# Edresson/VoiceSplit

Measured on AMD Instinct MI355X. Metric: utterances/sec (3 s clips, B=64/GPU) fwd+bwd, channels-last bf16 activations / tape, bf16 MFMA, fp32 accumulate / statistics / master weights, higher is better.
Workload: dtype bf16 (conv activations and tape stored as bf16; bf16 MFMA operands in the convs, the LSTM / head contractions and the BPTT, f16 operands in the forward recurrence; fp32 accumulate, BatchNorm statistics, gate arithmetic / cell state, loss head, master weights)

## Files before the change

include/voicesplit_hip.h:

```cpp
#ifndef VOICESPLIT_HIP_H
#define VOICESPLIT_HIP_H

#include <stddef.h>
#include <stdint.h>

#ifdef __cplusplus
extern "C" {
#endif
#if defined(__GNUC__)
#pragma GCC visibility push(default)
#endif

#define VS_ABI_VERSION 11

#define VS_ACT_RELU 0
#define VS_ACT_MISH 1
#define VS_ACT_NONE 2
#define VS_ACT_SIGMOID 3

#define VS_MATH_FP32 0
#define VS_MATH_F16X3 1
#define VS_MATH_BF16 2

#define VS_BN_EVAL 0
// ... 257 lines not shown
                     int conv_act, int bn_mode, void* tape, size_t tape_bytes, float* mask, void* stream);

int vs_backward(const vs_dims* dims, const vs_params* params, const float* x, const float* dvec,
                int conv_act, int bn_mode, void* tape, size_t tape_bytes,
                const float* mask, const float* dmask, const vs_grads* grads, void* stream);

int vs_conv64_pack_dgrad(const float* w, float* packed, int KT, int KF, void* stream);
size_t vs_conv64_wgrad_partial_floats(int KT, int KF);
int vs_conv64_wgrad(const float* dz, const float* in, float* partials, float* dw,
                    int B, int T, int F, int KT, int KF, int dil, void* stream);
int vs_conv64_wgrad_f16x3(const float* dz, const float* in, float* partials, float* dw, float* scratch8,
                          int B, int T, int F, int KT, int KF, int dil, void* stream);
int vs_set_wgrad_kernel(int mode);
int vs_set_conv_kernel(int mode);
int vs_set_lstm_kernel(int mode);

enum vs_option {
  VS_OPT_FWD_PROLOGUE = 0,
  VS_OPT_HEAD_LEAF_SIDE = 1,
  VS_OPT_FEAT_ROWS = 2,
  VS_OPT_HEAD_BWD_GEMM = 3,
  VS_OPT_ABLATION = 4,
  VS_OPT_DETERMINISTIC = 5,
  VS_OPT_COUNT = 6
};
int vs_set_option(int option, int value);
int vs_get_option(int option);

int vs_lstm_status(const vs_dims* dims, const void* tape, size_t tape_bytes, const void* workspace, size_t workspace_bytes, void* stream);

int vs_set_backward_overlap(int on);
int vs_bn_act_bwd(const float* da, const float* z, float* dz, int C, long long R, int L, int act, int bn_mode,
                  const float* scale, const float* shift, const float* mean, const float* invstd,
                  float* dgamma, float* dbeta, float* dbias, double* stats, float* coef, void* stream);
int vs_bn_act_bwd_first(const float* da, const float* z, const float* x, float* xpad, int B, int T, int F, int act, int bn_mode,
                        const float* scale, const float* shift, const float* mean, const float* invstd,
                        float* dgamma, float* dbeta, float* dbias, float* dw, double* stats, float* coef, double* acc, void* stream);
int vs_conv_last_dgrad(const float* dz, const float* w, float* din, int B, int T, int F, void* stream);
int vs_conv_last_wgrad_blocks(void);
int vs_conv_last_wgrad(const float* dz, const float* in, float* partials , float* dw,
                       int B, int T, int F, void* stream);
int vs_conv_first_wgrad(const float* dz, const float* x, double* acc, float* dw, int B, int T, int F, void* stream);
int vs_gemm(int layout_a, int layout_w, const float* A, int lda, const float* W, int ldw, float* C, int ldc,
            int M, int N, int K, const float* bias, const float* gate, int ldg, int a_relu, int w_relu, int act,
            int accumulate, int w_shift, int w_group, int splits, float* partials, void* stream);
int vs_gemm_f16x3(int layout_a, int layout_w, const float* A, int lda, const float* W, int ldw, float* C, int ldc,
                  int M, int N, int K, const float* bias, const float* gate, int ldg, int a_relu, int w_relu, int act,
// ... 123 lines not shown
```

voicesplit_amd/_lib.py:

```python
import ctypes
import os
from ctypes import POINTER, Structure, c_char_p, c_float, c_int, c_longlong, c_size_t, c_void_p

_HERE = os.path.dirname(os.path.abspath(__file__))
LIB_PATH = os.path.join(_HERE, "libvoicesplit_hip.so")

ACT_RELU, ACT_MISH, ACT_NONE, ACT_SIGMOID = 0, 1, 2, 3
BN_EVAL, BN_TRAIN = 0, 1
MATH_FP32, MATH_F16X3, MATH_BF16 = 0, 1, 2
PROF_SLOTS = 29
PROF_NAMES = ("cnn1", "cnn2", "cnn3", "cnn4", "cnn5", "cnn6", "cnn7", "cnn8", "lstm_gemm", "lstm_rec", "head",
              "fwd_bn", "bwd_head", "bwd_lstm_rec", "bwd_lstm_gemm", "bwd_bn",
              "wgrad_cnn2", "wgrad_cnn3", "wgrad_cnn4", "wgrad_cnn5", "wgrad_cnn6", "wgrad_cnn7",
              "dgrad_cnn2", "dgrad_cnn3", "dgrad_cnn4", "dgrad_cnn5", "dgrad_cnn6", "dgrad_cnn7", "bwd_edge")
ABI_VERSION = 11


class VsDims(Structure):
    _fields_ = [(n, c_int) for n in ("B", "T", "F", "E", "H", "FC1", "FC2", "math")]


class VsConvLayer(Structure):
    _fields_ = [(n, c_void_p) for n in ("weight", "bias", "bn_weight", "bn_bias",
                                        "bn_running_mean", "bn_running_var")]
# ... 215 lines not shown


def load(path: str = None) -> ctypes.CDLL:
    global _lib
    if _lib is not None and path is None:
        return _lib
    path = path or LIB_PATH
    if not os.path.isfile(path):
        raise VoiceSplitHipError(
            f"{path} not found: build it with `python -c 'import __graft_entry__ as g; g.build()'` "
            f"or `make -C voicesplit_amd/csrc`. There is no PyTorch/CPU fallback for this path.")
    lib = ctypes.CDLL(path)
    for name, (restype, argtypes) in SIGNATURES.items():
        fn = getattr(lib, name)
        fn.restype = restype
        fn.argtypes = argtypes
    if lib.vs_abi_version() != ABI_VERSION:
        raise VoiceSplitHipError(f"{path}: ABI version {lib.vs_abi_version()} != {ABI_VERSION}; rebuild")
    _apply_env_options(lib)
    _lib = lib
    return lib


OPTIONS = {"FWD_PROLOGUE": 0, "HEAD_LEAF_SIDE": 1, "FEAT_ROWS": 2, "HEAD_BWD_GEMM": 3, "ABLATION": 4, "DETERMINISTIC": 5}
_ENV_OPTIONS = {
    "VOICESPLIT_FWD_PROLOGUE": ("FWD_PROLOGUE", int),
    "VOICESPLIT_HEAD_LEAF_SIDE": ("HEAD_LEAF_SIDE", int),
    "VOICESPLIT_FEAT_ROWS": ("FEAT_ROWS", int),
    "VOICESPLIT_HEAD_BWD_GEMM": ("HEAD_BWD_GEMM", int),
    "VOICESPLIT_ABLATION": ("ABLATION", int),
    "VOICESPLIT_DETERMINISTIC": ("DETERMINISTIC", int),
}


def _apply_env_options(lib):
    for var, (name, conv) in _ENV_OPTIONS.items():
        v = os.environ.get(var)
        if v is None or v == "":
            continue
        try:
            value = conv(v)
        except ValueError as err:
            raise VoiceSplitHipError(f"{var}={v}: not a value of this switch ({err})") from None
        if lib.vs_set_option(OPTIONS[name], value) != 0:
            msg = lib.vs_last_error()
            raise VoiceSplitHipError(f"{var}={v}: {msg.decode() if msg else 'rejected by vs_set_option'}")


def set_option(name: str, value: int):
    lib = load()
    prev = lib.vs_get_option(OPTIONS[name])
    check(lib.vs_set_option(OPTIONS[name], int(value)), f"vs_set_option({name})")
    return prev

# ... 10 lines not shown
```

voicesplit_amd/csrc/capi.hip:

```cpp
#include <stdarg.h>
#include <stdlib.h>
#include <string.h>

#include "../../include/voicesplit_hip.h"
#include "vs_internal.h"

static thread_local char g_err[512] = "";

void vs_set_error(const char* fmt, ...) {
  va_list ap;
  va_start(ap, fmt);
  vsnprintf(g_err, sizeof(g_err), fmt, ap);
  va_end(ap);
}

int g_vs_options[VS_OPT_COUNT] = { 1,  1,  1,  1,  0,  0};
thread_local unsigned* g_vs_turn = nullptr;

namespace {
struct Prof {
  bool on = false;
  int max_calls = 0;
  int calls[VS_PROF_SLOTS] = {0};
  hipEvent_t* ev = nullptr;
} g_prof;

}

VsProfScope::VsProfScope(int slot, hipStream_t s_) : s(s_), idx(-1) {
  if (!g_prof.on || g_prof.calls[slot] >= g_prof.max_calls) return;
  idx = (g_prof.calls[slot]++ * VS_PROF_SLOTS + slot) * 2;
  (void)hipEventRecord(g_prof.ev[idx], s);
}
VsProfScope::~VsProfScope() { if (idx >= 0) (void)hipEventRecord(g_prof.ev[idx + 1], s); }

extern "C" {

int vs_abi_version(void) { return VS_ABI_VERSION; }

// ... 396 lines not shown
```

voicesplit_amd/csrc/gemm_bf16.hip:

```cpp
#include <stdlib.h>

#include <type_traits>

#include "vs_internal.h"

namespace {

typedef unsigned u4v __attribute__((ext_vector_type(4)));
typedef short s4v __attribute__((ext_vector_type(4)));
typedef short s8v __attribute__((ext_vector_type(8)));
typedef __attribute__((address_space(3))) unsigned char lds_byte;
typedef __attribute__((address_space(3))) const u4v lds_u4v;

__device__ u4v g_gemm_zero_page[4];

constexpr int TM = 256, TN = 256, BK = 64;
constexpr int A_BYTES = TM * BK * 2;
constexpr int B_BYTES = TN * BK * 2;
constexpr int STAGE_BYTES = A_BYTES + B_BYTES;
constexpr int NSTAGE = 2;
constexpr int WA = 8, WB = 8;

struct GemmBf16Args {
  const unsigned short* A; int lda;
  const unsigned short* B; int ldb;
  float* C; int ldc;
  float* C2; int split_m;
  int M, N, K;
  const float* rowbias; int ldrb, group;
  int accumulate;
  int tiles_m, tiles_n, band;
  const float* gate; int ldg;
  int vec_ok;
};

__device__ __forceinline__ void glds16(const void* gsrc, unsigned lds_dst) {
  unsigned keep;
  asm volatile("s_mov_b32 %0, m0\n\ts_mov_b32 m0, %2\n\ts_nop 0\n\tglobal_load_lds_dwordx4 %1, off\n\ts_mov_b32 m0, %0"
               : "=&s"(keep) : "v"(gsrc), "s"(lds_dst) : "memory");
}
__device__ __forceinline__ vs_bf16x8 frag_of(s4v lo, s4v hi) {
  const s8v v = {lo[0], lo[1], lo[2], lo[3], hi[0], hi[1], hi[2], hi[3]};
  return __builtin_bit_cast(vs_bf16x8, v);
}
__device__ __forceinline__ s4v ds_read_tr16(unsigned addr) {
  return __builtin_amdgcn_ds_read_tr16_b64_v4i16((__attribute__((address_space(3))) s4v*)(uintptr_t)addr);
}

template <bool KMAJOR, int R>
struct Operand {
  static_assert(R == 256, "the lane decomposition below is for 256-row operand tiles");
  static constexpr int CHUNKS = R / 8 / 4;
  struct LaneDma { unsigned off[2]; int line; int col[2]; };
  __device__ static __forceinline__ LaneDma lane_dma(int ld, int wave, int lane) {
    LaneDma L;
    if (!KMAJOR) {
// ... 187 lines not shown
        const float* rb = g.rowbias ? g.rowbias + (size_t)(m / g.group) * g.ldrb : nullptr;
#pragma unroll
        for (int b = 0; b < WB; ++b) {
          const int n = tn * TN + wn * 128 + b * 16 + i;
          if (n < g.N) {
            float v = acc[a][b][r];
            if (rb) v += rb[n];
            if (g.accumulate) v += crow[n];
            if (g.gate) v = g.gate[(size_t)m * g.ldg + n] > 0.f ? v : 0.f;
            crow[n] = v;
          }
        }
      }
  }
}

__device__ __forceinline__ f32x4 acc_read(const f32x4& t) {
  f32x4 v;
  asm volatile("v_accvgpr_read_b32 %0, %4\n\tv_accvgpr_read_b32 %1, %5\n\tv_accvgpr_read_b32 %2, %6\n\tv_accvgpr_read_b32 %3, %7"
               : "=v"(v[0]), "=v"(v[1]), "=v"(v[2]), "=v"(v[3]) : "a"(t[0]), "a"(t[1]), "a"(t[2]), "a"(t[3]));
  return v;
}

template <bool AK, bool BK_, int DR, int ABL = 0>
__global__ __launch_bounds__(256, 1)
void gemm_bf16_il_kernel(GemmBf16Args g) {
  __shared__ __attribute__((aligned(16))) unsigned char smem[NSTAGE * STAGE_BYTES];
  using OA = Operand<AK, TM>;
  using OB = Operand<BK_, TN>;
  const int lane = threadIdx.x & 63;
  const int wave = __builtin_amdgcn_readfirstlane(threadIdx.x >> 6);
  const int wm = wave >> 1, wn = wave & 1;
  const unsigned lds0 = (unsigned)(uintptr_t)(const lds_byte*)smem;
  const int nk = (g.K + BK - 1) / BK;

  const int per = (int)(gridDim.x >> 3);
  const int ntiles = g.tiles_m * g.tiles_n;
  const int tpx = (ntiles + 7) / 8;
  const int xcd = (int)(blockIdx.x & 7), slot = (int)(blockIdx.x >> 3);
  auto tile_id = [&](int j) { return xcd * tpx + slot + j * per; };
  auto tile_ok = [&](int j) { const int t = tile_id(j); return slot + j * per < tpx && t < ntiles; };

  int pj = 0, pk = 0, ptm = 0, ptn = 0;
  bool plive = tile_ok(0) && tile_of(g, tile_id(0), ptm, ptn);
  int pstage = 0;
  const unsigned fbA = AK ? (OA::frag_base(lane) ^ (unsigned)((wm * 8) << 5)) : (OA::frag_base(lane) + (unsigned)(wm * 128 * 128));
  const unsigned fbB = BK_ ? (OB::frag_base(lane) ^ (unsigned)((wn * 8) << 5)) : (OB::frag_base(lane) + (unsigned)(wn * 128 * 128));
  const typename OA::LaneDma la = OA::lane_dma(g.lda, wave, lane);
  const typename OB::LaneDma lb = OB::lane_dma(g.ldb, wave, lane);
  const unsigned pitchA = OA::chunk_pitch(g.lda), pitchB = OB::chunk_pitch(g.ldb);
  const unsigned kstepA = AK ? (unsigned)BK * (unsigned)g.lda * 2u : (unsigned)BK * 2u;
  const unsigned kstepB = BK_ ? (unsigned)BK * (unsigned)g.ldb * 2u : (unsigned)BK * 2u;
  const bool feed = g.accumulate >= 0;
  u4v dA = OA::tile_desc(g.A, g.lda, g.M, g.K, ptm * TM, 0, plive && feed), dB = OB::tile_desc(g.B, g.ldb, g.N, g.K, ptn * TN, 0, plive && feed);
  unsigned soffA = 0, soffB = 0;
  unsigned dstA = lds0 + (unsigned)(wave * 1024);
  auto dma_load = [&](unsigned voff, const u4v& desc, unsigned soff) {
    asm volatile("buffer_load_dwordx4 %0, %1, %2 offen lds" :: "v"(voff), "s"(desc), "s"(soff) : "memory");
  };
  auto adv = [&](u4v& d, unsigned step) {
    const unsigned long long b = (((unsigned long long)d[1] << 32) | d[0]) + step;
    d[0] = (unsigned)b;
    d[1] = (unsigned)(b >> 32);
    d[2] -= step;
  };
  auto pf_done = [&]() {
    pstage ^= 1;
    dstA = lds0 + (unsigned)(pstage * STAGE_BYTES) + (unsigned)(wave * 1024);
    if (++pk == nk) {
      pk = 0;
      ++pj;
      plive = tile_ok(pj) && tile_of(g, tile_id(pj), ptm, ptn);
      dA = OA::tile_desc(g.A, g.lda, g.M, g.K, ptm * TM, 0, plive && feed);
      dB = OB::tile_desc(g.B, g.ldb, g.N, g.K, ptn * TN, 0, plive && feed);
    }
  };
  if (plive) {
#pragma unroll
    for (int c = 0; c < 8; ++c) {
      asm volatile("s_mov_b32 m0, %0\n\ts_nop 0" :: "s"(dstA + (unsigned)(c * 4096)) : "memory");
      dma_load(AK ? la.off[c & 1] : la.off[0], dA, soffA);
      soffA += pitchA;
      asm volatile("s_mov_b32 m0, %0\n\ts_nop 0" :: "s"(dstA + (unsigned)(A_BYTES + c * 4096)) : "memory");
      dma_load(BK_ ? lb.off[c & 1] : lb.off[0], dB, soffB);
      soffB += pitchB;
    }
    soffA = soffB = 0;
    adv(dA, kstepA);
    adv(dB, kstepB);
    pf_done();
  }

  int cstage = 0;
  vs_bf16x8 bf[2][WB], afc, afn;
  asm volatile("s_waitcnt vmcnt(0)" ::: "memory");
  __builtin_amdgcn_s_barrier();
  for (int j = 0; tile_ok(j); ++j) {
    int tm, tn;
    if (!tile_of(g, tile_id(j), tm, tn)) break;
    f32x4 acc[WA][WB];
#pragma unroll
    for (int a = 0; a < WA; ++a)
#pragma unroll
      for (int b = 0; b < WB; ++b) acc[a][b] = f32x4{0.f, 0.f, 0.f, 0.f};
    {
      unsigned fa = lds0 + (unsigned)(cstage * STAGE_BYTES) + fbA, fb = lds0 + (unsigned)(cstage * STAGE_BYTES + A_BYTES) + fbB;
      asm volatile("" : "+v"(fa), "+v"(fb));
#pragma unroll
      for (int b = 0; b < WB; ++b) bf[0][b] = OB::frag(fb, b * 16, 0);
      afc = OA::frag(fa, 0, 0);
      afn = afc;
    }
    for (int ks = 0; ks < nk; ++ks) {
      const unsigned lv = (unsigned)__builtin_amdgcn_readfirstlane(plive ? 1 : 0);
      const unsigned stepA = (feed ? lv : 0u) * kstepA, stepB = (feed ? lv : 0u) * kstepB;
      unsigned fa = lds0 + (unsigned)(cstage * STAGE_BYTES) + fbA, fb = lds0 + (unsigned)(cstage * STAGE_BYTES + A_BYTES) + fbB;
      unsigned fan = lds0 + (unsigned)((cstage ^ 1) * STAGE_BYTES) + fbA, fbn = lds0 + (unsigned)((cstage ^ 1) * STAGE_BYTES + A_BYTES) + fbB;
      asm volatile("" : "+v"(fa), "+v"(fb), "+v"(fan), "+v"(fbn));
      const unsigned dstB = dstA + (unsigned)A_BYTES;
      __builtin_amdgcn_sched_barrier(0);
      auto row = [&](auto RC) {
        constexpr int R = decltype(RC)::value;
        constexpr int kh = R >> 3, a = R & 7;
        if (R == 15) {
          if (!(ABL & 2)) {
            asm volatile("s_waitcnt vmcnt(0) lgkmcnt(0)" ::: "memory");
            __builtin_amdgcn_s_barrier();
          }
          __builtin_amdgcn_sched_barrier(0);
        }
#pragma unroll
        for (int b = 0; b < WB; ++b) {
          asm volatile("v_mfma_f32_16x16x32_bf16 %0, %2, %1, %0" : "+a"(acc[a][b]) : "v"(afc), "v"(bf[kh][b]));
          if (ABL & 1) {
          } else if (R < 15) {
            if (b == 0) afn = (a + 1 < WA) ? OA::frag(fa, (a + 1) * 16, kh) : OA::frag(fa, 0, 1);
            if (kh == 0 && b == 1) bf[1][a] = OB::frag(fb, a * 16, 1);
          } else {
            bf[0][b] = OB::frag(fbn, b * 16, 0);
            if (b == WB - 1) afn = OA::frag(fan, 0, 0);
          }
          if (kh == 0 && DR == 8) {
            if (b == 2) asm volatile("s_add_i32 m0, %0, %1" :: "s"(dstA), "n"(a * 4096) : "scc", "memory");
            if (b == 3) dma_load(AK ? la.off[a & 1] : la.off[0], dA, soffA);
            if (b == 4) { soffA += pitchA; asm volatile("s_add_i32 m0, %0, %1" :: "s"(dstB), "n"(a * 4096) : "scc", "memory"); }
            if (b == 5) dma_load(BK_ ? lb.off[a & 1] : lb.off[0], dB, soffB);
            if (b == 6) soffB += pitchB;
          } else if (kh == 0 && DR == 4) {
            if (a < 4) {
              constexpr int c0 = (2 * a) & 7, c1 = (2 * a + 1) & 7;
              if (b == 0) asm volatile("s_add_i32 m0, %0, %1" :: "s"(dstA), "n"(c0 * 4096) : "scc", "memory");
              if (b == 1) { dma_load(AK ? la.off[c0 & 1] : la.off[0], dA, soffA); soffA += pitchA; }
              if (b == 2) asm volatile("s_add_i32 m0, %0, %1" :: "s"(dstB), "n"(c0 * 4096) : "scc", "memory");
              if (b == 3) { dma_load(BK_ ? lb.off[c0 & 1] : lb.off[0], dB, soffB); soffB += pitchB; }
              if (b == 4) asm volatile("s_add_i32 m0, %0, %1" :: "s"(dstA), "n"(c1 * 4096) : "scc", "memory");
              if (b == 5) { dma_load(AK ? la.off[c1 & 1] : la.off[0], dA, soffA); soffA += pitchA; }
              if (b == 6) asm volatile("s_add_i32 m0, %0, %1" :: "s"(dstB), "n"(c1 * 4096) : "scc", "memory");
              if (b == 7) { dma_load(BK_ ? lb.off[c1 & 1] : lb.off[0], dB, soffB); soffB += pitchB; }
            }
          } else {
            if (a == 0 && b == 2) adv(dA, stepA);
            if (a == 1 && b == 2) adv(dB, stepB);
          }
          __builtin_amdgcn_sched_barrier(0);
        }
        afc = afn;
      };
      row(std::integral_constant<int, 0>{});  row(std::integral_constant<int, 1>{});  row(std::integral_constant<int, 2>{});
      row(std::integral_constant<int, 3>{});  row(std::integral_constant<int, 4>{});  row(std::integral_constant<int, 5>{});
// ... 4 lines not shown
      soffA = soffB = 0;
      if (lv) pf_done();
      cstage ^= 1;
    }
    asm volatile("s_nop 15\n\ts_nop 15" ::: "memory");
    const int i = lane & 15, gq = lane >> 4;
    const bool whole = g.vec_ok && tm * TM + TM <= g.M && tn * TN + TN <= g.N;
    const int n0 = tn * TN + wn * 128 + 4 * gq;
    auto bias_ptr = [&](int a) -> const float* {
      int m = tm * TM + wm * 128 + a * 16 + i;
      m = m < g.M ? m : g.M - 1;
      return g.rowbias + (size_t)(m / g.group) * g.ldrb + n0;
    };
    f32x4 bias_nx[WB];
    if (whole && g.rowbias) {
      const float* rb0 = bias_ptr(0);
#pragma unroll
      for (int b = 0; b < WB; ++b) bias_nx[b] = *reinterpret_cast<const f32x4*>(rb0 + 16 * b);
    }
#pragma unroll
    for (int a = 0; a < WA; ++a) {
      const int m = tm * TM + wm * 128 + a * 16 + i;
      const int mc = m < g.M ? m : g.M - 1;
      float* crow = ((g.C2 && mc >= g.split_m) ? g.C2 + (size_t)(mc - g.split_m) * g.ldc : g.C + (size_t)mc * g.ldc) + n0;
      const float* rb = g.rowbias ? g.rowbias + (size_t)(mc / g.group) * g.ldrb + n0 : nullptr;
      if (whole) {
        f32x4 v[WB];
#pragma unroll
        for (int b = 0; b < WB; ++b) v[b] = acc_read(acc[a][b]);
        if (rb) {
#pragma unroll
          for (int b = 0; b < WB; ++b) v[b] += bias_nx[b];
          if (a + 1 < WA) {
            const float* rbn = bias_ptr(a + 1);
#pragma unroll
            for (int b = 0; b < WB; ++b) bias_nx[b] = *reinterpret_cast<const f32x4*>(rbn + 16 * b);
          }
        }
        if (g.accumulate > 0) {
#pragma unroll
          for (int b = 0; b < WB; ++b) v[b] += *reinterpret_cast<const f32x4*>(crow + 16 * b);
        }
        if (g.gate) {
          const float* gr = g.gate + (size_t)mc * g.ldg + n0;
#pragma unroll
          for (int b = 0; b < WB; ++b) {
            const f32x4 gt = *reinterpret_cast<const f32x4*>(gr + 16 * b);
// ... 51 lines not shown
      const f4 a0 = __builtin_nontemporal_load(p0), b0 = __builtin_nontemporal_load(p0 + 1);
      const f4 a1 = __builtin_nontemporal_load(p1), b1 = __builtin_nontemporal_load(p1 + 1);
      conv(i, a0, b0);
      conv(i + stride, a1, b1);
    }
    if (i < total) {
      const f4* p0 = addr(i);
      conv(i, __builtin_nontemporal_load(p0), __builtin_nontemporal_load(p0 + 1));
    }
    return;
  }
  for (long long i = (long long)blockIdx.x * 256 + threadIdx.x; i < total; i += (long long)gridDim.x * 256) {
    const long long r = i / groups;
    const int k0 = (int)(i - r * groups) * 8;
    const float* p = src + r * ld + k0;
    float x[8];
#pragma unroll
    for (int e = 0; e < 8; ++e) x[e] = (k0 + e < K) ? p[e] : 0.f;
    const u4v o = {vs_pack_bf16(x[0], x[1]), vs_pack_bf16(x[2], x[3]), vs_pack_bf16(x[4], x[5]), vs_pack_bf16(x[6], x[7])};
    *reinterpret_cast<u4v*>(dst + r * Kp + k0) = o;
  }
}

int gemm_cus() {
  int dev = 0, v = 0;
  if (hipGetDevice(&dev) != hipSuccess) return 256;
  if (hipDeviceGetAttribute(&v, hipDeviceAttributeMultiprocessorCount, dev) != hipSuccess || v <= 0) v = 256;
  return v;
}

}

int vs_cvt_rows_bf16_impl(const float* src, long long rows, int K, int ld, void* dst, int Kp, hipStream_t stream) {
  VS_REQUIRE(src && dst && rows > 0 && K > 0 && ld >= K && Kp >= K && Kp % 8 == 0, "cvt_rows_bf16: bad argument");
  const long long total = rows * (Kp >> 3);
  const long long nb = (total + 255) / 256;
  const long long ccap = 1LL << 24;
  const bool vec = K % 8 == 0 && ld % 4 == 0 && (reinterpret_cast<uintptr_t>(src) & 15) == 0 && (reinterpret_cast<uintptr_t>(dst) & 15) == 0;
  if (vec) hipLaunchKernelGGL(cvt_rows_bf16_kernel<true>, dim3((unsigned)(nb < ccap ? nb : ccap)), dim3(256), 0, stream, src, rows, K, ld,
                              reinterpret_cast<unsigned short*>(dst), Kp);
  else
  hipLaunchKernelGGL(cvt_rows_bf16_kernel<false>, dim3((unsigned)(nb < ccap ? nb : ccap)), dim3(256), 0, stream, src, rows, K, ld,
                     reinterpret_cast<unsigned short*>(dst), Kp);
  VS_LAUNCH_CHECK();
  return 0;
}

int vs_gemm_bf16_impl(int a_kmajor, int b_kmajor, const void* A, int lda, const void* B, int ldb, float* C, int ldc, float* C2, int split_m,
                      int M, int N, int K, const float* rowbias, int ldrb, int group, int accumulate, hipStream_t stream,
                      const float* gate, int ldg) {
  VS_REQUIRE(A && B && C && M > 0 && N > 0 && K > 0, "gemm_bf16: bad argument");
  VS_REQUIRE(lda % 8 == 0 && ldb % 8 == 0 && (reinterpret_cast<uintptr_t>(A) & 15) == 0 && (reinterpret_cast<uintptr_t>(B) & 15) == 0,
             "gemm_bf16: operands must be 16-byte aligned with ld a multiple of 8");
  VS_REQUIRE(!rowbias || (group > 0 && ldrb >= N), "gemm_bf16: rowbias needs group > 0 and ldrb >= N");
  VS_REQUIRE(!gate || (ldg >= N && !C2), "gemm_bf16: gate needs ldg >= N and a single output");
  VS_REQUIRE(a_kmajor || lda >= (K + BK - 1) / BK * BK, "gemm_bf16: row-form A must be padded to a multiple of %d in k", BK);
  VS_REQUIRE(b_kmajor || ldb >= (K + BK - 1) / BK * BK, "gemm_bf16: row-form B must be padded to a multiple of %d in k", BK);
  GemmBf16Args g{reinterpret_cast<const unsigned short*>(A), lda, reinterpret_cast<const unsigned short*>(B), ldb, C, ldc, C2, split_m,
                 M, N, K, rowbias, ldrb, group > 0 ? group : 1, accumulate, (M + TM - 1) / TM, (N + TN - 1) / TN, 8, gate, ldg, 0};
  g.vec_ok = N % 4 == 0 && ldc % 4 == 0 && (reinterpret_cast<uintptr_t>(C) & 15) == 0 && (!C2 || (reinterpret_cast<uintptr_t>(C2) & 15) == 0) &&
             (!rowbias || (ldrb % 4 == 0 && (reinterpret_cast<uintptr_t>(rowbias) & 15) == 0)) &&
             (!gate || (ldg % 4 == 0 && (reinterpret_cast<uintptr_t>(gate) & 15) == 0));
  static int cus = gemm_cus();
  const long long ntiles = (long long)g.tiles_m * g.tiles_n;
  long long nwg = cus / 8 * 8;
  if (nwg > (ntiles + 7) / 8 * 8) nwg = (ntiles + 7) / 8 * 8;
  if (nwg < 8) nwg = 8;
  const dim3 grid((unsigned)nwg), block(256);
  const int form = (!a_kmajor && !b_kmajor) ? 0 : (!a_kmajor && b_kmajor) ? 1 : (a_kmajor && b_kmajor) ? 2 : 3;
  VS_REQUIRE(form != 3, "gemm_bf16: the col x row form is not used by the path");
  if (g.vec_ok) {
#ifdef VS_ABLATION
    const int abl = vs_opt(VS_OPT_ABLATION);
    if (abl == 9) g.accumulate = -1;
    if (abl >= 1 && abl <= 3 && form == 0) {
      if (abl == 1) hipLaunchKernelGGL((gemm_bf16_il_kernel<false, false, 8, 1>), grid, block, 0, stream, g);
      else if (abl == 2) hipLaunchKernelGGL((gemm_bf16_il_kernel<false, false, 8, 2>), grid, block, 0, stream, g);
      else hipLaunchKernelGGL((gemm_bf16_il_kernel<false, false, 8, 3>), grid, block, 0, stream, g);
      VS_LAUNCH_CHECK();
      return 0;
    }
#endif
    if (form == 0) hipLaunchKernelGGL((gemm_bf16_il_kernel<false, false, 8>), grid, block, 0, stream, g);
    else if (form == 1) hipLaunchKernelGGL((gemm_bf16_il_kernel<false, true, 8>), grid, block, 0, stream, g);
    else hipLaunchKernelGGL((gemm_bf16_il_kernel<true, true, 8>), grid, block, 0, stream, g);
    VS_LAUNCH_CHECK();
    return 0;
  }
  if (form == 0) hipLaunchKernelGGL((gemm_bf16_kernel<false, false, 1>), grid, block, 0, stream, g);
  else if (form == 1) hipLaunchKernelGGL((gemm_bf16_kernel<false, true, 2>), grid, block, 0, stream, g);
  else hipLaunchKernelGGL((gemm_bf16_kernel<true, true, 2>), grid, block, 0, stream, g);
  VS_LAUNCH_CHECK();
  return 0;
// ... 2 lines not shown
```

voicesplit_amd/csrc/train.hip:

```cpp
#include <mutex>
#include <stdlib.h>
#include <string.h>

#include "../../include/voicesplit_hip.h"
#include "vs_internal.h"

namespace {

constexpr int kSplitK = 16;

inline size_t max3(size_t a, size_t b, size_t c) { return a > b ? (a > c ? a : c) : (b > c ? b : c); }

int tape_layout(const vs_dims* d, vs_tape_layout* L) {
  if (int rc = vs_check_dims_impl(d)) return rc;
  memset(L, 0, sizeof(*L));
  const size_t B = d->B, T = d->T, F = d->F, H = d->H, M = B * T;
  size_t off = 0;
  auto take = [&](size_t bytes) { size_t o = off; off = align_up(off + bytes); return o; };
  const size_t act = B * 64 * T * F * (d->math == VS_MATH_BF16 ? 2 : 4);
  for (int l = 0; l < 7; ++l) { L->z[l] = take(d->math == VS_MATH_BF16 && l == 0 ? 256 : act); L->a[l] = take(act); }
  L->z8 = take(M * 8 * F * 4);
  L->feat = take(M * 8 * F * 4);
  L->bn_scale = take(8 * 64 * 4);
  L->bn_shift = take(8 * 64 * 4);
  L->bn_mean = take(8 * 64 * 4);
  L->bn_invstd = take(8 * 64 * 4);
  L->gates = take(M * 8 * H * 4);
  L->cstate = take(M * 2 * H * 4);
  L->lstm_out = take(M * 2 * H * 4);
  L->fc1_out = take(M * (size_t)d->FC1 * 4);
  L->dlogits = take(M * (size_t)d->FC2 * 4);
  L->dfc1 = take(M * (size_t)d->FC1 * 4);
  L->dlstm_out = take(M * 2 * H * 4);
  L->dsum = take(B * 8 * H * 4);
  L->dfeat = take(M * 8 * F * 4);
  L->grad0 = take(act);
  L->grad1 = take(act);
  L->dvbias = take(B * 8 * H * 4);
  for (int i = 0; i < 6; ++i) L->conv_packed[i] = take(vs_conv64_packed_floats(kMid[i].kt, kMid[i].kf) * 4);
  L->pack_tmp = take(vs_conv64_packed_floats(5, 5) * 4);
  L->lstm_packed = take(vs_lstm_packed_floats(d->H) * 4);
  L->lstm_packed_t = take(vs_lstm_packed_t_floats(d->H) * 4);
  L->lstm_state = take(vs_lstm_state_floats(d->B, d->H) * 4);
  L->lstm_bwd_state = take(vs_lstm_bwd_state_floats(d->B, d->H) * 4);
  L->consts = take(128 * 4);
  L->bn_stats = take((size_t)VS_BN_STAT_SLOTS * 64 * 2 * 8);
  L->bn_coef = take(3 * 64 * 4);
  L->first_acc = take((64 + VS_FIRST_BWD_SCRATCH_DOUBLES) * 8);
  L->colsum_tmp = take(2 * B * max3(8 * H, d->FC1, d->FC2) * 4);
  size_t part = vs_conv64_wgrad_partial_floats(5, 5);
  part = max3(part, vs_conv64_wgrad_partial_floats(7, 1), (size_t)vs_conv_last_wgrad_blocks() * 512);
  part = max3(part, (size_t)kSplitK * d->FC2 * d->FC1, (size_t)kSplitK * d->FC1 * 2 * H);
  part = max3(part, (size_t)kSplitK * 4 * H * H, (size_t)0);
  L->partials = take(part * 4);
  L->conv_scales = take(16 * VS_SCALE_SLOT_FLOATS * 4);
  L->gemm_scales = take(32 * 4);
  L->lstm_bf16 = take(d->math == VS_MATH_BF16 ? vs_lstm_bf16_layout((long long)M, 8 * (int)F, (int)H).total : 256);
  L->det_turn = take(VS_TURN_WORDS * 4 + (size_t)VS_BN_STAT_SLOTS * 576 * 8);
  for (int i = 0; i < 6; ++i) L->conv_packed_t[i] = take(vs_conv64_packed_floats(kMid[i].kt, kMid[i].kf) * 4);
  L->total_bytes = off;
  return 0;
}

int check_tape(const vs_dims* d, void* tape, size_t bytes, vs_tape_layout* L) {
  if (int rc = tape_layout(d, L)) return rc;
  VS_REQUIRE(tape != nullptr, "tape is NULL");
  VS_REQUIRE((reinterpret_cast<uintptr_t>(tape) & 255) == 0, "tape must be 256-byte aligned");
  VS_REQUIRE(bytes >= L->total_bytes, "tape too small: %zu < %zu bytes", bytes, L->total_bytes);
  return 0;
}

int check_params(const vs_params* p) {
  VS_REQUIRE(p != nullptr, "params is NULL");
  for (int l = 0; l < 8; ++l) {
    const vs_conv_layer& c = p->conv[l];
    VS_REQUIRE(c.weight && c.bias && c.bn_weight && c.bn_bias && c.bn_running_mean && c.bn_running_var,
               "conv layer %d has a NULL parameter", l + 1);
  }
  for (int dir = 0; dir < 2; ++dir)
    VS_REQUIRE(p->w_ih[dir] && p->w_hh[dir] && p->b_ih[dir] && p->b_hh[dir], "NULL LSTM parameter (dir %d)", dir);
// ... 363 lines not shown
                                      st.B, st.T, st.H, st.stream, st.d->math);
}

int lstm_leaves(const Step& st, const SideJoin& sj, const float* dvec, const vs_grads* g) {
  hipStream_t ls = sj.to();
  const vs_params* p = st.p;
  const vs_tape_layout& L = st.L;
  const int B = st.B, T = st.T, H = st.H, M = st.M, K8 = st.K8, KE = st.KE, E = st.d->E;
  const bool f16x3 = st.d->math == VS_MATH_F16X3;
  float* dxg = st.at<float>(L.gates);
  float* dsum = st.at<float>(L.dsum);
  float* feat = st.at<float>(L.feat);
  float* lstm_out = st.at<float>(L.lstm_out);
  float* tmp = st.at<float>(L.colsum_tmp);
  float* gsc = st.at<float>(L.gemm_scales);
  char* bfb = st.at<char>(L.lstm_bf16);
  auto dwih_bf16 = [&]() -> int {
    return vs_gemm_bf16_impl(1, 1, bfb + st.lb.dxg, 8 * H, bfb + st.lb.feat, st.lb.Kp, g->w_ih[0], KE, g->w_ih[1], 4 * H, 8 * H, K8, M, nullptr, 0, 1, 0, ls);
  };
  const bool wih_last = sj.side != nullptr;
  VsProfScope ps(VS_PROF_BWD_LSTM_GEMM, ls);
  if (int rc = vs_colsum_impl(dxg, 8 * H, B, T, 8 * H, dsum, 8 * H, ls)) return rc;
  if (int rc = vs_colsum_impl(dsum, 8 * H, 1, B, 8 * H, tmp, 8 * H, ls)) return rc;
  for (int dir = 0; dir < 2; ++dir) {
    VS_CHECK_HIP(hipMemcpyAsync(g->b_ih[dir], tmp + (size_t)dir * 4 * H, sizeof(float) * 4 * H, hipMemcpyDeviceToDevice, ls));
    VS_CHECK_HIP(hipMemcpyAsync(g->b_hh[dir], tmp + (size_t)dir * 4 * H, sizeof(float) * 4 * H, hipMemcpyDeviceToDevice, ls));
    const float* dxg_d = dxg + (size_t)dir * 4 * H;
    if (st.nhwc) {
      if (dir == 0 && !wih_last) { if (int rc = dwih_bf16()) return rc; }
    } else if (f16x3) {
      if (int rc = vs_gemm_f16x3_impl(1, 1, dxg_d, 8 * H, feat, nullptr, 0x7fffffff, K8, g->w_ih[dir], KE, 4 * H, K8, M,
                                      nullptr, nullptr, nullptr, 0, 1, nullptr, 0, 0, 0, VS_ACT_NONE, 0, gsc + 8, gsc, ls, st.d->math)) return rc;
    } else {
      if (int rc = vs_gemm_general_impl(1, 1, dxg_d, 8 * H, feat, nullptr, 0x7fffffff, K8, g->w_ih[dir], KE, 4 * H, K8, M,
                                        nullptr, nullptr, nullptr, 0, 1, nullptr, 0, 0, 0, VS_ACT_NONE, 0, 0, 0, 1, nullptr, ls)) return rc;
    }
    if (int rc = vs_gemm_general_impl(1, 1, dsum + (size_t)dir * 4 * H, 8 * H, dvec, nullptr, 0x7fffffff, E, g->w_ih[dir] + K8, KE,
                                      4 * H, E, B, nullptr, nullptr, nullptr, 0, 1, nullptr, 0, 0, 0, VS_ACT_NONE, 0, 0, 0, 1, nullptr, ls)) return rc;
    if (int rc = (st.nhwc ? vs_gemm_general_bf16_impl : vs_gemm_general_impl)(1, 1, dxg_d, 8 * H, lstm_out + (size_t)dir * H, nullptr, 0x7fffffff, 2 * H,
                                      g->w_hh[dir], H, 4 * H, H, M, nullptr, nullptr, nullptr, 0, 1, nullptr, 0, 0, 0, VS_ACT_NONE, 0,
                                      dir ? 1 : -1, T, kSplitK, st.part, ls)) return rc;
    if (g->dvec) {
      if (int rc = vs_gemm_general_impl(0, 1, dsum + (size_t)dir * 4 * H, 8 * H, p->w_ih[dir] + K8, nullptr, 0x7fffffff, KE, g->dvec, E,
                                        B, E, 4 * H, nullptr, nullptr, nullptr, 0, 1, nullptr, 0, 0, 0, VS_ACT_NONE, dir, 0, 0, 1, nullptr, ls)) return rc;
    }
  }
  if (st.nhwc && wih_last) { if (int rc = dwih_bf16()) return rc; }
  return 0;
}

int dfeat_and_leaves(const Step& st, SideJoin& sj, const float* dvec, const vs_grads* g) {
  const vs_params* p = st.p;
  const vs_tape_layout& L = st.L;
  hipStream_t stream = st.stream;
  const int H = st.H, M = st.M, K8 = st.K8, KE = st.KE;
  const bool f16x3 = st.d->math == VS_MATH_F16X3;
  float* dxg = st.at<float>(L.gates);
  float* dfeat = st.at<float>(L.dfeat);
  float* gsc = st.at<float>(L.gemm_scales);
  char* bfb = st.at<char>(L.lstm_bf16);
  {
// ... 278 lines not shown
```

voicesplit_amd/csrc/vs_internal.h:

```cpp
#pragma once
#include "vs_common.h"

struct VsProfScope {
  hipStream_t s; int idx;
  VsProfScope(int slot, hipStream_t s);
  ~VsProfScope();
};

extern int g_vs_options[VS_OPT_COUNT];
inline int vs_opt(int o) { return g_vs_options[o]; }
extern thread_local unsigned* g_vs_turn;
struct VsTurnScope {
  unsigned* prev;
  explicit VsTurnScope(unsigned* t) : prev(g_vs_turn) { g_vs_turn = t; }
  ~VsTurnScope() { g_vs_turn = prev; }
};
inline int vs_det_grid(int nb, int cus = 256) { return (g_vs_turn && nb > cus) ? cus : nb; }

constexpr float kBnEps = 1e-5f;
constexpr float kBnMomentum = 0.1f;
struct Spec { int kt, kf, dil; };
constexpr Spec kMid[6] = {{7, 1, 1}, {5, 5, 1}, {5, 5, 2}, {5, 5, 4}, {5, 5, 8}, {5, 5, 16}};
inline size_t align_up(size_t x) { return (x + 255) & ~size_t(255); }
template <typename T>
// ... 161 lines not shown
int vs_conv_first_wgrad_impl(const float* dz, const float* x, double* acc, float* dw, int B, int T, int F, hipStream_t);
int vs_reduce_partials_impl(const float* part, int G, int n, float* out, hipStream_t);
int vs_gemm_general_impl(int layout_a, int layout_w, const float* A, int lda, const float* W, const float* W_hi,
                         int n_split, int ldw, float* C, int ldc, int M, int N, int K,
                         const float* bias1, const float* bias2, const float* rowbias, int ldrb, int group,
                         const float* gate, int ldg, int a_relu, int w_relu, int act, int accumulate,
                         int w_shift, int w_group, int splits, float* partials, hipStream_t);
int vs_gemm_general_bf16_impl(int layout_a, int layout_w, const float* A, int lda, const float* W, const float* W_hi,
                         int n_split, int ldw, float* C, int ldc, int M, int N, int K,
                         const float* bias1, const float* bias2, const float* rowbias, int ldrb, int group,
                         const float* gate, int ldg, int a_relu, int w_relu, int act, int accumulate,
                         int w_shift, int w_group, int splits, float* partials, hipStream_t);
int vs_gemm_nt_impl(const float*, int, const float*, int, float*, int, int, int, int, const float*, const float*, const float*, int, int, int, int, hipStream_t);
bool vs_head_fused_supported(int K1, int FC1, int FC2);
size_t vs_head_fused_packed_bytes(int K1, int FC1, int FC2);
int vs_head_fused_pack_impl(const float* w1, const float* b1, const float* w2, const float* b2, int K1, int FC1, int FC2, void* packed, hipStream_t);
int vs_head_fused_impl(const float* lstm_out, const void* packed, float* h1_out, float* logits, float* mask,
                       int M, int K1, int FC1, int FC2, hipStream_t);
int vs_gemm_nt_bf16_impl(const float*, int, const float*, int, float*, int, int, int, int, const float*, const float*, const float*, int, int, int, int, hipStream_t);
int vs_gemm_nt2_impl(const float*, int, const float*, const float*, int, int, float*, int, int, int, int, const float*, const float*, const float*, int, int, int, int, hipStream_t);
int vs_cvt_rows_bf16_impl(const float* src, long long rows, int K, int ld, void* dst, int Kp, hipStream_t);
int vs_gemm_bf16_impl(int a_kmajor, int b_kmajor, const void* A, int lda, const void* B, int ldb, float* C, int ldc, float* C2, int split_m,
                      int M, int N, int K, const float* rowbias, int ldrb, int group, int accumulate, hipStream_t,
                      const float* gate = nullptr, int ldg = 0);
struct VsLstmBf16Layout { size_t feat, wih, dxg, total; int Kp; };
inline VsLstmBf16Layout vs_lstm_bf16_layout(long long M, int K, int H) {
  VsLstmBf16Layout L;
  L.Kp = (K + 63) / 64 * 64;
  L.feat = 0;
  L.wih = align_up((size_t)M * L.Kp * 2);
  L.dxg = L.wih + align_up((size_t)8 * H * L.Kp * 2);
  L.total = L.dxg + align_up((size_t)M * 8 * H * 2);
  return L;
}
int vs_lstm_pack_impl(const float*, const float*, float*, int, hipStream_t, int math = VS_MATH_CODE_FP32);
struct VsLstmCarry {
  const float* state_in;
  float* state_out;
  int keep;
};
int vs_bilstm_recurrent_impl(const float* xg, const float* wp, float* state, float* out, float* gates_save, float* c_save,
                             int B, int T, int H, hipStream_t, int math = VS_MATH_CODE_FP32,
                             const int* lengths = nullptr ,
                             const float* rowbias = nullptr ,
                             int K = 1,
                             const VsLstmCarry* carry = nullptr );
int vs_lstm_carry_check(int math, int H, int T, int keep, const float* state_out, const char* what);
// ... 11 lines not shown
```

Baseline: 1450.

## Add split-K col x col bf16 GEMM with shifted-B operand for LSTM dW_hh

Adds a split-K variant of the bf16 MFMA GEMM kernel. Work items are distributed as (tile, K-chunk) pairs across all CUs, and per-split partials are reduced by a new fold kernel. A shifted-B mode masks the frame at each utterance boundary so the recurrent weight gradient can use the previous or next hidden state directly. The backward LSTM now converts lstm_out to bf16 and computes dW_hh through this path instead of the general split-K GEMM, aiming to fill the GPU for a small-tile, long-K contraction. The cost is an extra conversion pass, a partials buffer plus fold kernel, and a larger workspace.

New measurement: 1454, median of 6. Within noise of the previous version (+0.3%).

```diff
diff --git a/include/voicesplit_hip.h b/include/voicesplit_hip.h
--- a/include/voicesplit_hip.h
+++ b/include/voicesplit_hip.h
@@ -303,7 +303,8 @@
   VS_OPT_HEAD_BWD_GEMM = 3,
   VS_OPT_ABLATION = 4,
   VS_OPT_DETERMINISTIC = 5,
-  VS_OPT_COUNT = 6
+  VS_OPT_GEMM_SPLITK_WGS = 6,
+  VS_OPT_COUNT = 7
 };
 int vs_set_option(int option, int value);
 int vs_get_option(int option);
diff --git a/voicesplit_amd/_lib.py b/voicesplit_amd/_lib.py
--- a/voicesplit_amd/_lib.py
+++ b/voicesplit_amd/_lib.py
@@ -261,7 +261,8 @@
     return lib
 
 
-OPTIONS = {"FWD_PROLOGUE": 0, "HEAD_LEAF_SIDE": 1, "FEAT_ROWS": 2, "HEAD_BWD_GEMM": 3, "ABLATION": 4, "DETERMINISTIC": 5}
+OPTIONS = {"FWD_PROLOGUE": 0, "HEAD_LEAF_SIDE": 1, "FEAT_ROWS": 2, "HEAD_BWD_GEMM": 3, "ABLATION": 4, "DETERMINISTIC": 5,
+           "GEMM_SPLITK_WGS": 6}
 _ENV_OPTIONS = {
     "VOICESPLIT_FWD_PROLOGUE": ("FWD_PROLOGUE", int),
     "VOICESPLIT_HEAD_LEAF_SIDE": ("HEAD_LEAF_SIDE", int),
@@ -269,6 +270,7 @@
     "VOICESPLIT_HEAD_BWD_GEMM": ("HEAD_BWD_GEMM", int),
     "VOICESPLIT_ABLATION": ("ABLATION", int),
     "VOICESPLIT_DETERMINISTIC": ("DETERMINISTIC", int),
+    "VOICESPLIT_GEMM_SPLITK_WGS": ("GEMM_SPLITK_WGS", int),
 }
 
 
diff --git a/voicesplit_amd/csrc/capi.hip b/voicesplit_amd/csrc/capi.hip
--- a/voicesplit_amd/csrc/capi.hip
+++ b/voicesplit_amd/csrc/capi.hip
@@ -14,7 +14,8 @@
   va_end(ap);
 }
 
-int g_vs_options[VS_OPT_COUNT] = { 1,  1,  1,  1,  0,  0};
+int g_vs_options[VS_OPT_COUNT] = { 1,  1,  1,  1,  0,  0,
+                                   0};
 thread_local unsigned* g_vs_turn = nullptr;
 
 namespace {
diff --git a/voicesplit_amd/csrc/gemm_bf16.hip b/voicesplit_amd/csrc/gemm_bf16.hip
--- a/voicesplit_amd/csrc/gemm_bf16.hip
+++ b/voicesplit_amd/csrc/gemm_bf16.hip
@@ -32,6 +32,8 @@
   int tiles_m, tiles_n, band;
   const float* gate; int ldg;
   int vec_ok;
+  float* part; int nsplit, kchunk;
+  int b_group, b_cross; float b_rcp;
 };
 
 __device__ __forceinline__ void glds16(const void* gsrc, unsigned lds_dst) {
@@ -265,17 +267,18 @@
   return v;
 }
 
-template <bool AK, bool BK_, int DR, int ABL = 0>
+template <bool AK, bool BK_, int DR, int ABL = 0, int SK = 0>
 __global__ __launch_bounds__(256, 1)
 void gemm_bf16_il_kernel(GemmBf16Args g) {
   __shared__ __attribute__((aligned(16))) unsigned char smem[NSTAGE * STAGE_BYTES];
   using OA = Operand<AK, TM>;
   using OB = Operand<BK_, TN>;
+  static_assert(SK == 0 || (AK && BK_ && DR == 8 && ABL == 0), "the split-K form is col x col");
   const int lane = threadIdx.x & 63;
   const int wave = __builtin_amdgcn_readfirstlane(threadIdx.x >> 6);
   const int wm = wave >> 1, wn = wave & 1;
   const unsigned lds0 = (unsigned)(uintptr_t)(const lds_byte*)smem;
-  const int nk = (g.K + BK - 1) / BK;
+  const int nk_all = (g.K + BK - 1) / BK;
 
   const int per = (int)(gridDim.x >> 3);
   const int ntiles = g.tiles_m * g.tiles_n;
@@ -283,9 +286,24 @@
   const int xcd = (int)(blockIdx.x & 7), slot = (int)(blockIdx.x >> 3);
   auto tile_id = [&](int j) { return xcd * tpx + slot + j * per; };
   auto tile_ok = [&](int j) { const int t = tile_id(j); return slot + j * per < tpx && t < ntiles; };
-
-  int pj = 0, pk = 0, ptm = 0, ptn = 0;
-  bool plive = tile_ok(0) && tile_of(g, tile_id(0), ptm, ptn);
+  auto item = [&](int j, int& tm, int& tn, int& s) -> bool {
+    if constexpr (SK != 0) {
+      const int it = (int)blockIdx.x + j * (int)gridDim.x;
+      if (it >= ntiles * g.nsplit) return false;
+      s = it / ntiles;
+      return tile_of(g, it - s * ntiles, tm, tn);
+    } else {
+      s = 0;
+      return tile_ok(j) && tile_of(g, tile_id(j), tm, tn);
+    }
+  };
+  auto steps_of = [&](int s) { return SK != 0 ? min(g.kchunk, nk_all - s * g.kchunk) : nk_all; };
+  auto kbeg_of = [&](int s) { return SK != 0 ? s * g.kchunk * BK : 0; };
+  auto kend_of = [&](int s) { return SK != 0 ? min(g.K, (s + 1) * g.kchunk * BK) : g.K; };
+
+  int pj = 0, pk = 0, ptm = 0, ptn = 0, ps = 0;
+  bool plive = item(0, ptm, ptn, ps);
+  int pnk = steps_of(ps);
   int pstage = 0;
   const unsigned fbA = AK ? (OA::frag_base(lane) ^ (unsigned)((wm * 8) << 5)) : (OA::frag_base(lane) + (unsigned)(wm * 128 * 128));
   const unsigned fbB = BK_ ? (OB::frag_base(lane) ^ (unsigned)((wn * 8) << 5)) : (OB::frag_base(lane) + (unsigned)(wn * 128 * 128));
@@ -295,7 +313,18 @@
   const unsigned kstepA = AK ? (unsigned)BK * (unsigned)g.lda * 2u : (unsigned)BK * 2u;
   const unsigned kstepB = BK_ ? (unsigned)BK * (unsigned)g.ldb * 2u : (unsigned)BK * 2u;
   const bool feed = g.accumulate >= 0;
-  u4v dA = OA::tile_desc(g.A, g.lda, g.M, g.K, ptm * TM, 0, plive && feed), dB = OB::tile_desc(g.B, g.ldb, g.N, g.K, ptn * TN, 0, plive && feed);
+  u4v dA = OA::tile_desc(g.A, g.lda, g.M, kend_of(ps), ptm * TM, kbeg_of(ps), plive && feed);
+  u4v dB = OB::tile_desc(g.B, g.ldb, g.N, kend_of(ps), ptn * TN, kbeg_of(ps), plive && feed);
+  int pkabs = kbeg_of(ps);
+  auto voffB = [&](int c) -> unsigned {
+    const unsigned off = BK_ ? lb.off[c & 1] : lb.off[0];
+    if constexpr (SK == 2) {
+      const int k = pkabs + 8 * c + lb.line;
+      const int q = (int)(((float)k + 0.5f) * g.b_rcp);
+      return (k - q * g.b_group == g.b_cross) ? 0x7FFFFFF0u : off;
+    }
+    return off;
+  };
   unsigned soffA = 0, soffB = 0;
   unsigned dstA = lds0 + (unsigned)(wave * 1024);
   auto dma_load = [&](unsigned voff, const u4v& desc, unsigned soff) {
@@ -310,12 +339,15 @@
   auto pf_done = [&]() {
     pstage ^= 1;
     dstA = lds0 + (unsigned)(pstage * STAGE_BYTES) + (unsigned)(wave * 1024);
-    if (++pk == nk) {
+    if (SK == 2) pkabs += BK;
+    if (++pk == pnk) {
       pk = 0;
       ++pj;
-      plive = tile_ok(pj) && tile_of(g, tile_id(pj), ptm, ptn);
-      dA = OA::tile_desc(g.A, g.lda, g.M, g.K, ptm * TM, 0, plive && feed);
-      dB = OB::tile_desc(g.B, g.ldb, g.N, g.K, ptn * TN, 0, plive && feed);
+      plive = item(pj, ptm, ptn, ps);
+      pnk = steps_of(ps);
+      pkabs = kbeg_of(ps);
+      dA = OA::tile_desc(g.A, g.lda, g.M, kend_of(ps), ptm * TM, kbeg_of(ps), plive && feed);
+      dB = OB::tile_desc(g.B, g.ldb, g.N, kend_of(ps), ptn * TN, kbeg_of(ps), plive && feed);
     }
   };
   if (plive) {
@@ -325,7 +357,7 @@
       dma_load(AK ? la.off[c & 1] : la.off[0], dA, soffA);
       soffA += pitchA;
       asm volatile("s_mov_b32 m0, %0\n\ts_nop 0" :: "s"(dstA + (unsigned)(A_BYTES + c * 4096)) : "memory");
-      dma_load(BK_ ? lb.off[c & 1] : lb.off[0], dB, soffB);
+      dma_load(voffB(c), dB, soffB);
       soffB += pitchB;
     }
     soffA = soffB = 0;
@@ -338,9 +370,10 @@
   vs_bf16x8 bf[2][WB], afc, afn;
   asm volatile("s_waitcnt vmcnt(0)" ::: "memory");
   __builtin_amdgcn_s_barrier();
-  for (int j = 0; tile_ok(j); ++j) {
-    int tm, tn;
-    if (!tile_of(g, tile_id(j), tm, tn)) break;
+  for (int j = 0;; ++j) {
+    int tm, tn, cs;
+    if (!item(j, tm, tn, cs)) break;
+    const int nk = steps_of(cs);
     f32x4 acc[WA][WB];
 #pragma unroll
     for (int a = 0; a < WA; ++a)
@@ -387,7 +420,7 @@
             if (b == 2) asm volatile("s_add_i32 m0, %0, %1" :: "s"(dstA), "n"(a * 4096) : "scc", "memory");
             if (b == 3) dma_load(AK ? la.off[a & 1] : la.off[0], dA, soffA);
             if (b == 4) { soffA += pitchA; asm volatile("s_add_i32 m0, %0, %1" :: "s"(dstB), "n"(a * 4096) : "scc", "memory"); }
-            if (b == 5) dma_load(BK_ ? lb.off[a & 1] : lb.off[0], dB, soffB);
+            if (b == 5) dma_load(voffB(a), dB, soffB);
             if (b == 6) soffB += pitchB;
           } else if (kh == 0 && DR == 4) {
             if (a < 4) {
@@ -438,7 +471,9 @@
     for (int a = 0; a < WA; ++a) {
       const int m = tm * TM + wm * 128 + a * 16 + i;
       const int mc = m < g.M ? m : g.M - 1;
-      float* crow = ((g.C2 && mc >= g.split_m) ? g.C2 + (size_t)(mc - g.split_m) * g.ldc : g.C + (size_t)mc * g.ldc) + n0;
+      float* crow;
+      if constexpr (SK != 0) crow = g.part + ((size_t)cs * g.M + mc) * g.N + n0;
+      else crow = ((g.C2 && mc >= g.split_m) ? g.C2 + (size_t)(mc - g.split_m) * g.ldc : g.C + (size_t)mc * g.ldc) + n0;
       const float* rb = g.rowbias ? g.rowbias + (size_t)(mc / g.group) * g.ldrb + n0 : nullptr;
       if (whole) {
         f32x4 v[WB];
@@ -536,6 +571,20 @@
   }
 }
 
+__global__ __launch_bounds__(256)
+void splitk_fold_kernel(const float* __restrict__ part, int nsplit, int M, int N, float* __restrict__ C, float* __restrict__ C2, int split_m, int ldc) {
+  const int n4 = N >> 2;
+  const long long i = (long long)blockIdx.x * 256 + threadIdx.x;
+  if (i >= (long long)M * n4) return;
+  const int m = (int)(i / n4), n = (int)(i - (long long)m * n4) * 4;
+  const size_t slice = (size_t)M * N;
+  const float* p = part + (size_t)m * N + n;
+  f32x4 v = *reinterpret_cast<const f32x4*>(p);
+  for (int s = 1; s < nsplit; ++s) v += *reinterpret_cast<const f32x4*>(p + s * slice);
+  float* crow = (C2 && m >= split_m) ? C2 + (size_t)(m - split_m) * ldc : C + (size_t)m * ldc;
+  *reinterpret_cast<f32x4*>(crow + n) = v;
+}
+
 int gemm_cus() {
   int dev = 0, v = 0;
   if (hipGetDevice(&dev) != hipSuccess) return 256;
@@ -560,9 +609,16 @@
   return 0;
 }
 
+bool vs_gemm_bf16_splitk_shape(int M, int N, int K, int ldc, const float* C, const float* C2) {
+  static int cus = gemm_cus();
+  const long long ntiles = (long long)((M + TM - 1) / TM) * ((N + TN - 1) / TN);
+  return M > 0 && N > 0 && K > 0 && K < (1 << 20) && ntiles * 2 <= cus && N % 4 == 0 && ldc % 4 == 0 && (reinterpret_cast<uintptr_t>(C) & 15) == 0 &&
+         (!C2 || (reinterpret_cast<uintptr_t>(C2) & 15) == 0);
+}
+
 int vs_gemm_bf16_impl(int a_kmajor, int b_kmajor, const void* A, int lda, const void* B, int ldb, float* C, int ldc, float* C2, int split_m,
                       int M, int N, int K, const float* rowbias, int ldrb, int group, int accumulate, hipStream_t stream,
-                      const float* gate, int ldg) {
+                      const float* gate, int ldg, float* partials, size_t part_floats, int b_shift, int b_group) {
   VS_REQUIRE(A && B && C && M > 0 && N > 0 && K > 0, "gemm_bf16: bad argument");
   VS_REQUIRE(lda % 8 == 0 && ldb % 8 == 0 && (reinterpret_cast<uintptr_t>(A) & 15) == 0 && (reinterpret_cast<uintptr_t>(B) & 15) == 0,
              "gemm_bf16: operands must be 16-byte aligned with ld a multiple of 8");
@@ -583,6 +639,39 @@
   const dim3 grid((unsigned)nwg), block(256);
   const int form = (!a_kmajor && !b_kmajor) ? 0 : (!a_kmajor && b_kmajor) ? 1 : (a_kmajor && b_kmajor) ? 2 : 3;
   VS_REQUIRE(form != 3, "gemm_bf16: the col x row form is not used by the path");
+  const bool splitk = form == 2 && !rowbias && !gate && !accumulate && vs_gemm_bf16_splitk_shape(M, N, K, ldc, C, C2);
+  VS_REQUIRE(!b_shift || (splitk && (b_shift == 1 || b_shift == -1) && b_group > 0 && K % b_group == 0 && (long long)K * ldb * 2 < 0x7FFF0000ll),
+             "gemm_bf16: a shifted B operand needs the split-K col x col form, a shift of +-1 frame and K a multiple of the group");
+  if (splitk) {
+    const int nk = (K + BK - 1) / BK;
+    const size_t slice = (size_t)M * N;
+    long long want = cus / ntiles;
+    if (want > nk) want = nk;
+    if (partials && (long long)(part_floats / slice) < want) want = (long long)(part_floats / slice);
+    VS_REQUIRE(want >= 1, "gemm_bf16: the split-K scratch is smaller than one %d x %d partial", M, N);
+    g.kchunk = (int)((nk + want - 1) / want);
+    g.nsplit = (nk + g.kchunk - 1) / g.kchunk;
+    float* tmp = nullptr;
+    if (!partials) VS_CHECK_HIP(hipMallocAsync(reinterpret_cast<void**>(&tmp), (size_t)g.nsplit * slice * sizeof(float), stream));
+    g.part = partials ? partials : tmp;
+    long long items = ntiles * g.nsplit, wgs = items < cus ? items : cus;
+    const int cap = vs_opt(VS_OPT_GEMM_SPLITK_WGS);
+    if (cap > 0 && wgs > ntiles * cap) wgs = ntiles * cap;
+    if (b_shift) {
+      g.B = reinterpret_cast<const unsigned short*>(B) + (long long)b_shift * ldb;
+      g.b_group = b_group;
+      g.b_cross = b_shift < 0 ? 0 : b_group - 1;
+      g.b_rcp = 1.0f / (float)b_group;
+      hipLaunchKernelGGL((gemm_bf16_il_kernel<true, true, 8, 0, 2>), dim3((unsigned)wgs), block, 0, stream, g);
+    } else {
+      hipLaunchKernelGGL((gemm_bf16_il_kernel<true, true, 8, 0, 1>), dim3((unsigned)wgs), block, 0, stream, g);
+    }
+    VS_LAUNCH_CHECK();
+    hipLaunchKernelGGL(splitk_fold_kernel, dim3((unsigned)((slice / 4 + 255) / 256)), dim3(256), 0, stream, g.part, g.nsplit, M, N, C, C2, split_m, ldc);
+    VS_LAUNCH_CHECK();
+    if (tmp) VS_CHECK_HIP(hipFreeAsync(tmp, stream));
+    return 0;
+  }
   if (g.vec_ok) {
 #ifdef VS_ABLATION
     const int abl = vs_opt(VS_OPT_ABLATION);
diff --git a/voicesplit_amd/csrc/train.hip b/voicesplit_amd/csrc/train.hip
--- a/voicesplit_amd/csrc/train.hip
+++ b/voicesplit_amd/csrc/train.hip
@@ -8,6 +8,7 @@
 namespace {
 
 constexpr int kSplitK = 16;
+constexpr int kHhRanges = 24;
 
 inline size_t max3(size_t a, size_t b, size_t c) { return a > b ? (a > c ? a : c) : (b > c ? b : c); }
 
@@ -51,11 +52,11 @@
   size_t part = vs_conv64_wgrad_partial_floats(5, 5);
   part = max3(part, vs_conv64_wgrad_partial_floats(7, 1), (size_t)vs_conv_last_wgrad_blocks() * 512);
   part = max3(part, (size_t)kSplitK * d->FC2 * d->FC1, (size_t)kSplitK * d->FC1 * 2 * H);
-  part = max3(part, (size_t)kSplitK * 4 * H * H, (size_t)0);
+  part = max3(part, (size_t)kSplitK * 4 * H * H, d->math == VS_MATH_BF16 ? (size_t)kHhRanges * 4 * H * H : (size_t)0);
   L->partials = take(part * 4);
   L->conv_scales = take(16 * VS_SCALE_SLOT_FLOATS * 4);
   L->gemm_scales = take(32 * 4);
-  L->lstm_bf16 = take(d->math == VS_MATH_BF16 ? vs_lstm_bf16_layout((long long)M, 8 * (int)F, (int)H).total : 256);
+  L->lstm_bf16 = take(d->math == VS_MATH_BF16 ? vs_lstm_bf16_layout((long long)M, 8 * (int)F, (int)H).total + align_up(M * 2 * H * 2) : 256);
   L->det_turn = take(VS_TURN_WORDS * 4 + (size_t)VS_BN_STAT_SLOTS * 576 * 8);
   for (int i = 0; i < 6; ++i) L->conv_packed_t[i] = take(vs_conv64_packed_floats(kMid[i].kt, kMid[i].kf) * 4);
   L->total_bytes = off;
@@ -465,6 +466,10 @@
   VsProfScope ps(VS_PROF_BWD_LSTM_GEMM, ls);
   if (int rc = vs_colsum_impl(dxg, 8 * H, B, T, 8 * H, dsum, 8 * H, ls)) return rc;
   if (int rc = vs_colsum_impl(dsum, 8 * H, 1, B, 8 * H, tmp, 8 * H, ls)) return rc;
+  char* hout_bf = bfb + st.lb.total;
+  const bool hh_bf16 = st.nhwc && H % 8 == 0 && vs_gemm_bf16_splitk_shape(4 * H, H, M, H, g->w_hh[0], g->w_hh[1]) &&
+                       (L.conv_scales - L.partials) / sizeof(float) >= (size_t)4 * H * H && (long long)M * 2 * H * 2 < 0x7FFF0000ll;
+  if (hh_bf16) { if (int rc = vs_cvt_rows_bf16_impl(lstm_out, M, 2 * H, 2 * H, hout_bf, 2 * H, ls)) return rc; }
   for (int dir = 0; dir < 2; ++dir) {
     VS_CHECK_HIP(hipMemcpyAsync(g->b_ih[dir], tmp + (size_t)dir * 4 * H, sizeof(float) * 4 * H, hipMemcpyDeviceToDevice, ls));
     VS_CHECK_HIP(hipMemcpyAsync(g->b_hh[dir], tmp + (size_t)dir * 4 * H, sizeof(float) * 4 * H, hipMemcpyDeviceToDevice, ls));
@@ -480,6 +485,11 @@
     }
     if (int rc = vs_gemm_general_impl(1, 1, dsum + (size_t)dir * 4 * H, 8 * H, dvec, nullptr, 0x7fffffff, E, g->w_ih[dir] + K8, KE,
                                       4 * H, E, B, nullptr, nullptr, nullptr, 0, 1, nullptr, 0, 0, 0, VS_ACT_NONE, 0, 0, 0, 1, nullptr, ls)) return rc;
+    if (hh_bf16) {
+      if (int rc = vs_gemm_bf16_impl(1, 1, bfb + st.lb.dxg + (size_t)dir * 4 * H * 2, 8 * H, hout_bf + (size_t)dir * H * 2, 2 * H, g->w_hh[dir], H,
+                                     nullptr, 0, 4 * H, H, M, nullptr, 0, 1, 0, ls, nullptr, 0, st.part, (L.conv_scales - L.partials) / sizeof(float),
+                                     dir ? 1 : -1, T)) return rc;
+    } else
     if (int rc = (st.nhwc ? vs_gemm_general_bf16_impl : vs_gemm_general_impl)(1, 1, dxg_d, 8 * H, lstm_out + (size_t)dir * H, nullptr, 0x7fffffff, 2 * H,
                                       g->w_hh[dir], H, 4 * H, H, M, nullptr, nullptr, nullptr, 0, 1, nullptr, 0, 0, 0, VS_ACT_NONE, 0,
                                       dir ? 1 : -1, T, kSplitK, st.part, ls)) return rc;
diff --git a/voicesplit_amd/csrc/vs_internal.h b/voicesplit_amd/csrc/vs_internal.h
--- a/voicesplit_amd/csrc/vs_internal.h
+++ b/voicesplit_amd/csrc/vs_internal.h
@@ -207,7 +207,9 @@
 int vs_cvt_rows_bf16_impl(const float* src, long long rows, int K, int ld, void* dst, int Kp, hipStream_t);
 int vs_gemm_bf16_impl(int a_kmajor, int b_kmajor, const void* A, int lda, const void* B, int ldb, float* C, int ldc, float* C2, int split_m,
                       int M, int N, int K, const float* rowbias, int ldrb, int group, int accumulate, hipStream_t,
-                      const float* gate = nullptr, int ldg = 0);
+                      const float* gate = nullptr, int ldg = 0,
+                      float* partials = nullptr, size_t part_floats = 0, int b_shift = 0, int b_group = 0);
+bool vs_gemm_bf16_splitk_shape(int M, int N, int K, int ldc, const float* C, const float* C2);
 struct VsLstmBf16Layout { size_t feat, wih, dxg, total; int Kp; };
 inline VsLstmBf16Layout vs_lstm_bf16_layout(long long M, int K, int H) {
   VsLstmBf16Layout L;
```
